# CVMI-Lab/DODA

Measured on AMD Instinct MI355X. Metric: active-voxels/sec fwd+bwd SparseConv U-Net, ScanNet 2cm, higher is better.
Workload: dtype bf16; 1 GPU; cfgs/scannet SparseConv U-Net training step (voxel pooling + fwd + CE + bwd + SGD), 2 cm voxels, 4 scenes/GPU x ~150000 active voxels, random-init weights; global_batch=4, voxels_per_gpu=601279, points_per_gpu=781042, parallelism=dp1, n_classes=20, grad_sync=deferred multi-layer wgrad + bucketed all-reduce, collectives=none (single process), prefetch_gate=off, grad_exchange=no process group

## Files before the change

### doda_amd/csrc/spconv_wwide.hip

```cpp
#include "wgrad_common.hpp"
#include "tilebook.hpp"
#include <string.h>
#include <algorithm>
#include <vector>

namespace {

constexpr int WW_WAVES = 16;
constexpr int WW_MO = (TB_K + WW_WAVES - 1) / WW_WAVES;
constexpr int WW_LIST_BYTES = TB_UMAX * 4;
constexpr int ww_stage_bytes(int ta, int tb) { return TB_T * 32 * tb + (TB_LMAX + 1) * 32 * ta; }
constexpr int WW_STAGE_MAX = ww_stage_bytes(3, 3);
constexpr int WW_SMEM = WW_LIST_BYTES + TB_LIDX_BYTES + WW_STAGE_MAX;
static_assert(WW_SMEM <= 160 * 1024, "one workgroup per CU");
static_assert(TB_T + 1 <= TB_LMAX + 1, "the dense fallback stages 256 rows into the row slots");

struct WwJob {
    const unsigned short *x, *dy;
    const int32_t *tbl;
    const void *tb;
    float *dw, *part;
    int ca, cb, ld, n_rows, nt, ta, tb_, n_sb, P, rpc, accumulate;
    int wg_end, red_end;
    int pad;
};

__device__ __forceinline__ s16x4 ww_tr(unsigned addr) {
    return __builtin_amdgcn_ds_read_tr16_b64_v4i16((__attribute__((address_space(3))) s16x4 *)(uintptr_t)addr);
}
__device__ __forceinline__ bf16x8 ww_frag(unsigned a_lo, unsigned a_hi) {
    const s16x4 lo = ww_tr(a_lo), hi = ww_tr(a_hi);
    return __builtin_bit_cast(bf16x8, __builtin_shufflevector(lo, hi, 0, 1, 2, 3, 4, 5, 6, 7));
}

template <int TA, int TB>
__device__ void ww_body(const WwJob &d, int local, unsigned char *smem) {
    constexpr int RA = 32 * TA, RB = 32 * TB;
    constexpr int CIS = 16 * TA, COS = 16 * TB, SLICE = TB_K * CIS * COS;
    const int tid = threadIdx.x, wid = __builtin_amdgcn_readfirstlane(tid >> 6);
    const int lane = tid & 63, i = lane & 15, g = lane >> 4, q4 = i >> 2, c4 = i & 3;
    const int slice = local / d.P, p = local - slice * d.P;
    const int sa = slice / d.n_sb, sb = slice - sa * d.n_sb;
    const int ca0 = sa * CIS, cb0 = sb * COS;
    const int r_begin = p * d.rpc, r_end = min(d.n_rows, r_begin + d.rpc);
    const int tile_begin = r_begin / TB_T, tile_end = (r_end - 1) / TB_T + 1;
    static_assert(ww_stage_bytes(TA, TB) <= WW_STAGE_MAX, "staging buffers");
    const int32_t *tb_ulist = (const int32_t *)d.tb;
    const uint32_t *tb_lidx = (const uint32_t *)(tb_ulist + (size_t)d.nt * TB_UMAX);
    const int32_t *tb_ucount = (const int32_t *)(tb_lidx + (size_t)d.nt * (TB_LIDX_BYTES / 4));

    int32_t *list_s = reinterpret_cast<int32_t *>(smem);
    const unsigned *lidx_s = reinterpret_cast<const unsigned *>(smem + WW_LIST_BYTES);
    unsigned char *dy_s = smem + WW_LIST_BYTES + TB_LIDX_BYTES;
    unsigned char *rows_s = dy_s + TB_T * RB;
    const unsigned dy_base = (unsigned)(uintptr_t)dy_s, rows_base = (unsigned)(uintptr_t)rows_s;

    f32x4 acc[WW_MO][TA][TB];
#pragma unroll
    for (int m = 0; m < WW_MO; ++m)
#pragma unroll
        for (int a = 0; a < TA; ++a)
#pragma unroll
            for (int b = 0; b < TB; ++b) acc[m][a][b] = (f32x4){0.f, 0.f, 0.f, 0.f};

    auto multiply = [&](bool dense, int only_o, int ks_begin, int ks_end) {
#pragma unroll 1
        for (int ks = ks_begin; ks < ks_end; ++ks) {
            const int r = 32 * ks + 8 * g + q4;
            bf16x8 bf[TB];
#pragma unroll
            for (int b = 0; b < TB; ++b) {
                const unsigned a0 = dy_base + (unsigned)(r * RB + b * 32 + c4 * 8);
                bf[b] = ww_frag(a0, a0 + 4u * RB);
            }
#pragma unroll
            for (int m = 0; m < WW_MO; ++m) {
                const int o = wid + WW_WAVES * m;
                if (o >= TB_K || (dense && o != only_o)) continue;
                unsigned s0, s1;
                if (dense) {
                    s0 = (unsigned)(r + 1);
                    s1 = (unsigned)(r + 5);
                } else {
                    const unsigned *pl = lidx_s + tb_lplane(o) * TB_T;
                    const unsigned sh = tb_lshift(o);
                    s0 = __builtin_amdgcn_ubfe(pl[tb_lpos(r)], sh, 10u);
                    s1 = __builtin_amdgcn_ubfe(pl[tb_lpos(r + 4)], sh, 10u);
                }
                const unsigned x0 = rows_base + s0 * RA + (unsigned)(c4 * 8), x1 = rows_base + s1 * RA + (unsigned)(c4 * 8);
#pragma unroll
                for (int a = 0; a < TA; ++a) {
                    const bf16x8 af = ww_frag(x0 + 32u * a, x1 + 32u * a);
#pragma unroll
                    for (int b = 0; b < TB; ++b)
                        acc[m][a][b] = __builtin_amdgcn_mfma_f32_16x16x32_bf16(af, bf[b], acc[m][a][b], 0, 0, 0);
                }
            }
        }
    };

    for (int e = tid; e < RA / 16; e += 1024) reinterpret_cast<u32x4 *>(rows_s)[e] = (u32x4){0u, 0u, 0u, 0u};
    for (int tile = tile_begin; tile < tile_end; ++tile) {
        const int t0 = tile * TB_T;
        const int ks_begin = max(0, (r_begin - t0) / 32), ks_end = min(TB_T / 32, (r_end - t0 + 31) / 32);
        const int ucount = tb_ucount[tile];
        const bool listed = ucount <= TB_LMAX;
        if (listed) {
            const int e = (tid & 3) * 256 + ((tid >> 7) & 7) * 32 + ((tid >> 2) & 31);
            list_s[e] = tb_ulist[(size_t)tile * TB_UMAX + tid];
            for (int v = tid; v < TB_LIDX_BYTES / 16; v += 1024)
                reinterpret_cast<u32x4 *>(smem + WW_LIST_BYTES)[v] =
                    reinterpret_cast<const u32x4 *>(tb_lidx + (size_t)tile * (TB_LIDX_BYTES / 4))[v];
        }
        for (int v = tid; v < TB_T * (RB / 16); v += 1024) {
            const int t = v / (RB / 16), f = v - t * (RB / 16);
            u32x4 val = (u32x4){0u, 0u, 0u, 0u};
            if (t0 + t < d.n_rows) val = *reinterpret_cast<const u32x4 *>(d.dy + (size_t)(t0 + t) * d.cb + cb0 + f * 8);
            *reinterpret_cast<u32x4 *>(dy_s + t * RB + f * 16) = val;
        }
        doda_sync();
        if (listed) {
            for (int v = tid; v < ucount * (RA / 16); v += 1024) {
                const int e = v / (RA / 16), f = v - e * (RA / 16);
                const int row = list_s[e];
                *reinterpret_cast<u32x4 *>(rows_s + (e + 1) * RA + f * 16) =
                    *reinterpret_cast<const u32x4 *>(d.x + (size_t)row * d.ca + ca0 + f * 8);
            }
            doda_sync();
            multiply(false, 0, ks_begin, ks_end);
            doda_sync();
        } else {
            for (int o = 0; o < TB_K; ++o) {
                for (int v = tid; v < TB_T * (RA / 16); v += 1024) {
                    const int t = v / (RA / 16), f = v - t * (RA / 16);
                    const int row = t0 + t < d.n_rows ? d.tbl[(size_t)o * d.ld + t0 + t] : -1;
                    u32x4 val = (u32x4){0u, 0u, 0u, 0u};
                    if (row >= 0) val = *reinterpret_cast<const u32x4 *>(d.x + (size_t)row * d.ca + ca0 + f * 8);
                    *reinterpret_cast<u32x4 *>(rows_s + (t + 1) * RA + f * 16) = val;
                }
                doda_sync();
                multiply(true, o, ks_begin, ks_end);
                doda_sync();
            }
        }
    }

    float *dst = d.part + (size_t)local * SLICE;
#pragma unroll
    for (int m = 0; m < WW_MO; ++m) {
        const int o = wid + WW_WAVES * m;
        if (o >= TB_K) continue;
#pragma unroll
        for (int a = 0; a < TA; ++a)
#pragma unroll
            for (int b = 0; b < TB; ++b)
#pragma unroll
                for (int r = 0; r < 4; ++r)
                    dst[((size_t)o * CIS + a * 16 + 4 * g + r) * COS + b * 16 + i] = acc[m][a][b][r];
    }
}

__global__ __launch_bounds__(1024) void wgrad_wide(const WwJob *__restrict__ jobs, int n_jobs) {
    __shared__ __attribute__((aligned(16))) unsigned char smem[WW_SMEM];
    const int j = find_job<WwJob, &WwJob::wg_end>(jobs, n_jobs, (int)blockIdx.x);
    const WwJob d = jobs[j];
    const int local = (int)blockIdx.x - (j == 0 ? 0 : jobs[j - 1].wg_end);
#define WW_CASE(A, B) if (d.ta == A && d.tb_ == B) { ww_body<A, B>(d, local, smem); return; }
    WW_SHAPES(WW_CASE)
#undef WW_CASE
}

__global__ __launch_bounds__(256) void wgrad_wide_reduce(const WwJob *__restrict__ jobs, int n_jobs) {
    const int j = find_job<WwJob, &WwJob::red_end>(jobs, n_jobs, (int)blockIdx.x);
    const WwJob d = jobs[j];
    const int CIS = 16 * d.ta, COS = 16 * d.tb_, SLICE = TB_K * CIS * COS;
    wgrad_fold((int)blockIdx.x - (j == 0 ? 0 : jobs[j - 1].red_end), d.P, (long long)TB_K * d.ca * d.cb / 4, SLICE / 4,
               reinterpret_cast<float4 *>(d.dw), d.accumulate, [&](long long q) {
        const long long e = 4 * q;
        const int co = (int)(e % d.cb), ci = (int)((e / d.cb) % d.ca), o = (int)(e / ((long long)d.ca * d.cb));
        const int slice = (ci / CIS) * d.n_sb + co / COS;
        return reinterpret_cast<const float4 *>(d.part + ((size_t)slice * d.P) * SLICE + ((size_t)o * CIS + ci % CIS) * COS + co % COS);
    });
}

}

namespace doda_wwide {

Plan plan(const doda_wgrad_job *jobs, const std::vector<int> &idx) {
    Plan pl;
    pl.n = (int)idx.size();
    std::vector<int> order;
    for (int k = 0; k < pl.n; ++k) order.push_back(k);
    std::stable_sort(order.begin(), order.end(), [&](int a, int b) { return jobs[idx[a]].n_rows > jobs[idx[b]].n_rows; });
    std::vector<WwJob> desc;
    for (int kk : order) {
        const doda_wgrad_job &j = jobs[idx[kk]];
        WwJob d;
        d.x = (const unsigned short *)j.a; d.dy = (const unsigned short *)j.b; d.tbl = j.tbl; d.tb = j.tilebook;
        d.dw = j.dw;
        d.ca = j.ca; d.cb = j.cb; d.ld = j.ld; d.n_rows = j.n_rows; d.nt = (j.n_rows + TB_T - 1) / TB_T;
        const WideGeo g = wwide_geo(j, doda_wgrad::switches());
        d.ta = g.ta; d.tb_ = g.tb; d.rpc = g.rpc; d.P = g.P;
        d.n_sb = j.cb / (16 * d.tb_);
        d.accumulate = (j.flags & DODA_WGRAD_ACCUMULATE) ? 1 : 0;
        d.part = (float *)(uintptr_t)pl.partial_bytes;
        pl.partial_bytes += g.partial_bytes;
        pl.wgs += g.blocks;
        d.wg_end = pl.wgs;
        pl.red_blocks += doda_wgrad::reduce_blocks((long long)TB_K * j.ca * j.cb / 4, d.P);
        d.red_end = pl.red_blocks;
        d.pad = 0;
        desc.push_back(d);
    }
    pl.desc_bytes = desc.size() * sizeof(WwJob);
    pl.desc.resize(pl.desc_bytes);
    if (pl.desc_bytes) memcpy(pl.desc.data(), desc.data(), pl.desc_bytes);
    return pl;
}

size_t desc_bytes_per_job() { return sizeof(WwJob); }

void write_desc(const Plan &p, char *part, void *desc) {
    if (p.desc_bytes) memcpy(desc, p.desc.data(), p.desc_bytes);
    WwJob *d = (WwJob *)desc;
    for (int k = 0; k < p.n; ++k) d[k].part = (float *)(part + (uintptr_t)d[k].part);
}

int launch(const Plan &p, const void *desc_dev, hipStream_t s) {
    doda_wgrad::trace("wgrad_wide", p.wgs, 1024, p.n);
    hipLaunchKernelGGL(wgrad_wide, dim3(p.wgs), dim3(1024), 0, s, (const WwJob *)desc_dev, p.n);
    doda_wgrad::trace("wgrad_wide_reduce", p.red_blocks, 256, p.n);
    hipLaunchKernelGGL(wgrad_wide_reduce, dim3(p.red_blocks), dim3(256), 0, s, (const WwJob *)desc_dev, p.n);
    return doda_check_launch();
}

}
```

### doda_amd/csrc/wgrad_common.hpp

```cpp
#pragma once
#include "wgrad_backends.hpp"

typedef float f32x4 __attribute__((ext_vector_type(4)));
typedef short s16x4 __attribute__((ext_vector_type(4)));
typedef __bf16 bf16x8 __attribute__((ext_vector_type(8)));
typedef unsigned int u32x4 __attribute__((ext_vector_type(4)));

namespace {

template <class J, int J::*END>
__device__ __forceinline__ int find_job(const J *jobs, int n_jobs, int blk) {
    int lo = 0, hi = n_jobs - 1;
    while (lo < hi) {
        const int mid = (lo + hi) >> 1;
        if (blk < jobs[mid].*END) hi = mid; else lo = mid + 1;
    }
    return lo;
}

__device__ __forceinline__ bf16x8 pack_hi16(const f32x4 &d0, const f32x4 &d1) {
    u32x4 r;
    r[0] = __builtin_amdgcn_perm(__float_as_uint(d0[1]), __float_as_uint(d0[0]), 0x07060302u);
    r[1] = __builtin_amdgcn_perm(__float_as_uint(d0[3]), __float_as_uint(d0[2]), 0x07060302u);
    r[2] = __builtin_amdgcn_perm(__float_as_uint(d1[1]), __float_as_uint(d1[0]), 0x07060302u);
    r[3] = __builtin_amdgcn_perm(__float_as_uint(d1[3]), __float_as_uint(d1[2]), 0x07060302u);
    return __builtin_bit_cast(bf16x8, r);
}

template <class Src>
__device__ __forceinline__ void wgrad_fold(int blk, int R, long long n_quad, long long stride, float4 *dw, int accumulate,
                                           Src src) {
    __shared__ float4 part[256];
    const int RL = doda_wgrad::reduce_lanes(R), EL = 256 / RL;
    const int el = (int)threadIdx.x % EL, rl = (int)threadIdx.x / EL;
    const long long q = (long long)blk * EL + el;
    float4 s = make_float4(0.f, 0.f, 0.f, 0.f);
    if (q < n_quad) {
        const float4 *p = src(q);
        for (int r = rl; r < R; r += RL) {
            const float4 v = p[(long long)r * stride];
            s.x += v.x; s.y += v.y; s.z += v.z; s.w += v.w;
        }
    }
    part[rl * EL + el] = s;
    doda_sync();
    if (rl == 0 && q < n_quad) {
        float4 t = part[el];
        for (int r = 1; r < RL; ++r) {
            const float4 v = part[r * EL + el];
            t.x += v.x; t.y += v.y; t.z += v.z; t.w += v.w;
        }
        if (accumulate) {
            const float4 old = dw[q];
            t.x += old.x; t.y += old.y; t.z += old.z; t.w += old.w;
        }
        dw[q] = t;
    }
}

}
```

Measured before the change: 138.3 million voxels/s.

## Pipeline wide wgrad tiles with async LDS DMA, double-buffered lists and faster job lookup

Gathered input rows for the next tile are now fetched into LDS with global_load_lds DMA requests interleaved with the current tile's MFMA loop. The tile lists are double-buffered, and the row area is split from both ends so two tiles' rows can coexist. The next tile's dy and lidx are prefetched into registers. It also adds a TA==1 loop order that reuses A fragments, a ballot-based job lookup, cheaper unsigned index math in the reduce, and a 4-way unrolled fold loop. The goal is to hide gather latency and cut barriers, at the cost of more registers, inline asm that manipulates m0, and a more intricate synchronization scheme.

```diff
diff --git a/doda_amd/csrc/spconv_wwide.hip b/doda_amd/csrc/spconv_wwide.hip
--- a/doda_amd/csrc/spconv_wwide.hip
+++ b/doda_amd/csrc/spconv_wwide.hip
@@ -9,11 +9,16 @@
 constexpr int WW_WAVES = 16;
 constexpr int WW_MO = (TB_K + WW_WAVES - 1) / WW_WAVES;
 constexpr int WW_LIST_BYTES = TB_UMAX * 4;
-constexpr int ww_stage_bytes(int ta, int tb) { return TB_T * 32 * tb + (TB_LMAX + 1) * 32 * ta; }
-constexpr int WW_STAGE_MAX = ww_stage_bytes(3, 3);
-constexpr int WW_SMEM = WW_LIST_BYTES + TB_LIDX_BYTES + WW_STAGE_MAX;
-static_assert(WW_SMEM <= 160 * 1024, "one workgroup per CU");
-static_assert(TB_T + 1 <= TB_LMAX + 1, "the dense fallback stages 256 rows into the row slots");
+constexpr int WW_SMEM = 160 * 1024;
+template <int TA, int TB>
+struct WwLds {
+    static constexpr int RA = 32 * TA, RB = 32 * TB;
+    static constexpr int LIST = 0, LIDX = 2 * WW_LIST_BYTES, DY = LIDX + TB_LIDX_BYTES, ROWS = DY + TB_T * RB;
+    static constexpr int SLOTS = (WW_SMEM - ROWS) / RA;
+    static constexpr int NDY = (TB_T * (RB / 16) + 1023) / 1024;
+    static_assert(SLOTS >= TB_LMAX + 1, "a full list fits the row area");
+    static_assert(TB_T + 1 <= SLOTS, "the dense fallback stages 256 rows into the row slots");
+};
 
 struct WwJob {
     const unsigned short *x, *dy;
@@ -33,9 +38,32 @@
     return __builtin_bit_cast(bf16x8, __builtin_shufflevector(lo, hi, 0, 1, 2, 3, 4, 5, 6, 7));
 }
 
+#define WW_GLOBAL __attribute__((address_space(1)))
+template <class T>
+__device__ __forceinline__ WW_GLOBAL T *ww_global(T *p) { return (WW_GLOBAL T *)p; }
+typedef const WW_GLOBAL u32x4 *ww_g128;
+
+__device__ __forceinline__ void ww_dma16(unsigned lds_base, const WW_GLOBAL void *src) {
+    unsigned keep;
+    asm volatile("s_mov_b32 %0, m0\n\t"
+                 "s_mov_b32 m0, %1\n\t"
+                 "s_nop 0\n\t"
+                 "global_load_lds_dwordx4 %2, off\n\t"
+                 "s_mov_b32 m0, %0"
+                 : "=&s"(keep) : "s"(lds_base), "v"(src) : "memory");
+}
+__device__ __forceinline__ void ww_dma_drain() { asm volatile("s_waitcnt vmcnt(0)" ::: "memory"); }
+
+__device__ __forceinline__ int ww_tid() {
+    int t = (int)threadIdx.x;
+    asm volatile("" : "+v"(t));
+    return t;
+}
+
 template <int TA, int TB>
 __device__ void ww_body(const WwJob &d, int local, unsigned char *smem) {
-    constexpr int RA = 32 * TA, RB = 32 * TB;
+    typedef WwLds<TA, TB> L;
+    constexpr int RA = L::RA, RB = L::RB, NDY = L::NDY;
     constexpr int CIS = 16 * TA, COS = 16 * TB, SLICE = TB_K * CIS * COS;
     const int tid = threadIdx.x, wid = __builtin_amdgcn_readfirstlane(tid >> 6);
     const int lane = tid & 63, i = lane & 15, g = lane >> 4, q4 = i >> 2, c4 = i & 3;
@@ -44,16 +72,19 @@
     const int ca0 = sa * CIS, cb0 = sb * COS;
     const int r_begin = p * d.rpc, r_end = min(d.n_rows, r_begin + d.rpc);
     const int tile_begin = r_begin / TB_T, tile_end = (r_end - 1) / TB_T + 1;
-    static_assert(ww_stage_bytes(TA, TB) <= WW_STAGE_MAX, "staging buffers");
     const int32_t *tb_ulist = (const int32_t *)d.tb;
     const uint32_t *tb_lidx = (const uint32_t *)(tb_ulist + (size_t)d.nt * TB_UMAX);
     const int32_t *tb_ucount = (const int32_t *)(tb_lidx + (size_t)d.nt * (TB_LIDX_BYTES / 4));
-
-    int32_t *list_s = reinterpret_cast<int32_t *>(smem);
-    const unsigned *lidx_s = reinterpret_cast<const unsigned *>(smem + WW_LIST_BYTES);
-    unsigned char *dy_s = smem + WW_LIST_BYTES + TB_LIDX_BYTES;
-    unsigned char *rows_s = dy_s + TB_T * RB;
-    const unsigned dy_base = (unsigned)(uintptr_t)dy_s, rows_base = (unsigned)(uintptr_t)rows_s;
+    const WW_GLOBAL unsigned short *gx = ww_global(d.x), *gdy = ww_global(d.dy);
+    const WW_GLOBAL int32_t *gtbl = ww_global(d.tbl);
+
+    const unsigned *lidx_s = reinterpret_cast<const unsigned *>(smem + L::LIDX);
+    unsigned char *dy_s = smem + L::DY;
+    unsigned char *rows_s = smem + L::ROWS;
+    const unsigned dy_base = (unsigned)(uintptr_t)dy_s;
+    const auto list_of = [&](int tile) { return reinterpret_cast<int32_t *>(smem + L::LIST + (tile & 1) * WW_LIST_BYTES); };
+    const auto rows_of = [&](int tile, int ucount) { return rows_s + ((tile & 1) ? (L::SLOTS - (ucount + 1)) * RA : 0); };
+    const auto list_e = [](int t) { return (t & 3) * 256 + ((t >> 7) & 7) * 32 + ((t >> 2) & 31); };
 
     f32x4 acc[WW_MO][TA][TB];
 #pragma unroll
@@ -63,20 +94,49 @@
 #pragma unroll
             for (int b = 0; b < TB; ++b) acc[m][a][b] = (f32x4){0.f, 0.f, 0.f, 0.f};
 
-    auto multiply = [&](bool dense, int only_o, int ks_begin, int ks_end) {
+    u32x4 p_lidx = (u32x4){0u, 0u, 0u, 0u}, p_dy[NDY];
+    const auto load_p1 = [&](int tile) {
+        const int tl = ww_tid();
+        if (tl < TB_LIDX_BYTES / 16) p_lidx = reinterpret_cast<ww_g128>(ww_global(tb_lidx) + (size_t)tile * (TB_LIDX_BYTES / 4))[tl];
+#pragma unroll
+        for (int k = 0; k < NDY; ++k) {
+            const int v = tl + 1024 * k, t = v / (RB / 16), f = v - t * (RB / 16);
+            p_dy[k] = (u32x4){0u, 0u, 0u, 0u};
+            if (v < TB_T * (RB / 16) && tile * TB_T + t < d.n_rows)
+                p_dy[k] = *reinterpret_cast<ww_g128>(gdy + (size_t)(tile * TB_T + t) * d.cb + cb0 + f * 8);
+        }
+    };
+    const auto store_p1 = [&]() {
+        const int tl = ww_tid();
+        if (tl < TB_LIDX_BYTES / 16) reinterpret_cast<u32x4 *>(smem + L::LIDX)[tl] = p_lidx;
+#pragma unroll
+        for (int k = 0; k < NDY; ++k) {
+            const int v = tl + 1024 * k;
+            if (v < TB_T * (RB / 16)) reinterpret_cast<u32x4 *>(dy_s)[v] = p_dy[k];
+        }
+    };
+    const auto request_rows = [&](const int32_t *list, unsigned char *rows, int n, int &vb) {
+        const int v = vb + (ww_tid() & 63);
+        if (v < n) {
+            const int e = v / (RA / 16), f = v - e * (RA / 16);
+            ww_dma16(__builtin_amdgcn_readfirstlane((unsigned)(uintptr_t)rows + (unsigned)(RA + 16 * vb)),
+                     gx + (size_t)list[e] * d.ca + ca0 + f * 8);
+        }
+        vb += 1024;
+    };
+
+    auto multiply = [&](bool dense, int only_o, int ks_begin, int ks_end, unsigned rows_base, const int32_t *next_list,
+                        unsigned char *next_rows, int n_next) {
+        int vb = 64 * wid;
 #pragma unroll 1
         for (int ks = ks_begin; ks < ks_end; ++ks) {
+            if (vb < n_next) request_rows(next_list, next_rows, n_next, vb);
             const int r = 32 * ks + 8 * g + q4;
-            bf16x8 bf[TB];
-#pragma unroll
-            for (int b = 0; b < TB; ++b) {
+            const auto b_frag = [&](int b) {
                 const unsigned a0 = dy_base + (unsigned)(r * RB + b * 32 + c4 * 8);
-                bf[b] = ww_frag(a0, a0 + 4u * RB);
-            }
-#pragma unroll
-            for (int m = 0; m < WW_MO; ++m) {
-                const int o = wid + WW_WAVES * m;
-                if (o >= TB_K || (dense && o != only_o)) continue;
+                return ww_frag(a0, a0 + 4u * RB);
+            };
+            const auto a_rows = [&](int o, unsigned *x0, unsigned *x1) {
                 unsigned s0, s1;
                 if (dense) {
                     s0 = (unsigned)(r + 1);
@@ -87,65 +147,116 @@
                     s0 = __builtin_amdgcn_ubfe(pl[tb_lpos(r)], sh, 10u);
                     s1 = __builtin_amdgcn_ubfe(pl[tb_lpos(r + 4)], sh, 10u);
                 }
-                const unsigned x0 = rows_base + s0 * RA + (unsigned)(c4 * 8), x1 = rows_base + s1 * RA + (unsigned)(c4 * 8);
-#pragma unroll
-                for (int a = 0; a < TA; ++a) {
-                    const bf16x8 af = ww_frag(x0 + 32u * a, x1 + 32u * a);
-#pragma unroll
-                    for (int b = 0; b < TB; ++b)
-                        acc[m][a][b] = __builtin_amdgcn_mfma_f32_16x16x32_bf16(af, bf[b], acc[m][a][b], 0, 0, 0);
+                *x0 = rows_base + s0 * RA + (unsigned)(c4 * 8);
+                *x1 = rows_base + s1 * RA + (unsigned)(c4 * 8);
+            };
+            if constexpr (TA == 1) {
+                bf16x8 af[WW_MO];
+                bool own[WW_MO];
+#pragma unroll
+                for (int m = 0; m < WW_MO; ++m) {
+                    const int o = wid + WW_WAVES * m;
+                    own[m] = o < TB_K && !(dense && o != only_o);
+                    if (!own[m]) continue;
+                    unsigned x0, x1;
+                    a_rows(o, &x0, &x1);
+                    af[m] = ww_frag(x0, x1);
+                }
+#pragma unroll
+                for (int b = 0; b < TB; ++b) {
+                    const bf16x8 bf = b_frag(b);
+#pragma unroll
+                    for (int m = 0; m < WW_MO; ++m)
+                        if (own[m]) acc[m][0][b] = __builtin_amdgcn_mfma_f32_16x16x32_bf16(af[m], bf, acc[m][0][b], 0, 0, 0);
+                }
+            } else {
+                bf16x8 bf[TB];
+#pragma unroll
+                for (int b = 0; b < TB; ++b) bf[b] = b_frag(b);
+#pragma unroll
+                for (int m = 0; m < WW_MO; ++m) {
+                    const int o = wid + WW_WAVES * m;
+                    if (o >= TB_K || (dense && o != only_o)) continue;
+                    unsigned x0, x1;
+                    a_rows(o, &x0, &x1);
+#pragma unroll
+                    for (int a = 0; a < TA; ++a) {
+                        const bf16x8 af = ww_frag(x0 + 32u * a, x1 + 32u * a);
+#pragma unroll
+                        for (int b = 0; b < TB; ++b)
+                            acc[m][a][b] = __builtin_amdgcn_mfma_f32_16x16x32_bf16(af, bf[b], acc[m][a][b], 0, 0, 0);
+                    }
                 }
             }
         }
+        while (vb < n_next) request_rows(next_list, next_rows, n_next, vb);
     };
 
-    for (int e = tid; e < RA / 16; e += 1024) reinterpret_cast<u32x4 *>(rows_s)[e] = (u32x4){0u, 0u, 0u, 0u};
+    bool have_p1 = false;
+    bool have_rows = false;
+    const auto count_of = [&](int tile) { return tile < tile_end ? ww_global(tb_ucount)[tile + (ww_tid() >> 31)] : TB_LMAX + 1; };
+    int ucount = count_of(tile_begin), ucount1 = count_of(tile_begin + 1);
     for (int tile = tile_begin; tile < tile_end; ++tile) {
         const int t0 = tile * TB_T;
         const int ks_begin = max(0, (r_begin - t0) / 32), ks_end = min(TB_T / 32, (r_end - t0 + 31) / 32);
-        const int ucount = tb_ucount[tile];
+        const bool next = tile + 1 < tile_end;
         const bool listed = ucount <= TB_LMAX;
-        if (listed) {
-            const int e = (tid & 3) * 256 + ((tid >> 7) & 7) * 32 + ((tid >> 2) & 31);
-            list_s[e] = tb_ulist[(size_t)tile * TB_UMAX + tid];
-            for (int v = tid; v < TB_LIDX_BYTES / 16; v += 1024)
-                reinterpret_cast<u32x4 *>(smem + WW_LIST_BYTES)[v] =
-                    reinterpret_cast<const u32x4 *>(tb_lidx + (size_t)tile * (TB_LIDX_BYTES / 4))[v];
-        }
-        for (int v = tid; v < TB_T * (RB / 16); v += 1024) {
-            const int t = v / (RB / 16), f = v - t * (RB / 16);
-            u32x4 val = (u32x4){0u, 0u, 0u, 0u};
-            if (t0 + t < d.n_rows) val = *reinterpret_cast<const u32x4 *>(d.dy + (size_t)(t0 + t) * d.cb + cb0 + f * 8);
-            *reinterpret_cast<u32x4 *>(dy_s + t * RB + f * 16) = val;
-        }
+        if (!have_p1) {
+            load_p1(tile);
+            const int tl = ww_tid();
+            list_of(tile)[list_e(tl)] = tb_ulist[(size_t)tile * TB_UMAX + tl];
+            if (next) list_of(tile + 1)[list_e(tl)] = tb_ulist[(size_t)(tile + 1) * TB_UMAX + tl];
+        }
+        store_p1();
         doda_sync();
         if (listed) {
-            for (int v = tid; v < ucount * (RA / 16); v += 1024) {
-                const int e = v / (RA / 16), f = v - e * (RA / 16);
-                const int row = list_s[e];
-                *reinterpret_cast<u32x4 *>(rows_s + (e + 1) * RA + f * 16) =
-                    *reinterpret_cast<const u32x4 *>(d.x + (size_t)row * d.ca + ca0 + f * 8);
+            unsigned char *rows = rows_of(tile, ucount);
+            if (!have_rows) {
+                const int tl = ww_tid();
+                if (tl < RA / 16) reinterpret_cast<u32x4 *>(rows)[tl] = (u32x4){0u, 0u, 0u, 0u};
+                const int32_t *list = list_of(tile);
+                for (int vb = 64 * wid; vb < ucount * (RA / 16);) request_rows(list, rows, ucount * (RA / 16), vb);
+                ww_dma_drain();
+                doda_sync();
             }
+            int next_list = -1;
+            if (next) load_p1(tile + 1);
+            const int count2 = count_of(tile + 2);
+            if (tile + 2 < tile_end) next_list = ww_global(tb_ulist)[(size_t)(tile + 2) * TB_UMAX + ww_tid()];
+            const bool stage = next && ucount1 <= TB_LMAX && ucount + ucount1 + 2 <= L::SLOTS;
+            unsigned char *rows1 = rows_of(tile + 1, ucount1);
+            if (stage && ww_tid() < RA / 16) reinterpret_cast<u32x4 *>(rows1)[ww_tid()] = (u32x4){0u, 0u, 0u, 0u};
+            multiply(false, 0, ks_begin, ks_end, (unsigned)(uintptr_t)rows, list_of(tile + 1), rows1,
+                     stage ? ucount1 * (RA / 16) : 0);
+            ww_dma_drain();
             doda_sync();
-            multiply(false, 0, ks_begin, ks_end);
-            doda_sync();
+            if (tile + 2 < tile_end) list_of(tile)[list_e(ww_tid())] = next_list;
+            have_p1 = next;
+            have_rows = stage;
+            ucount = ucount1;
+            ucount1 = count2;
         } else {
             for (int o = 0; o < TB_K; ++o) {
-                for (int v = tid; v < TB_T * (RA / 16); v += 1024) {
+                for (int v = ww_tid(); v < TB_T * (RA / 16); v += 1024) {
                     const int t = v / (RA / 16), f = v - t * (RA / 16);
-                    const int row = t0 + t < d.n_rows ? d.tbl[(size_t)o * d.ld + t0 + t] : -1;
+                    const int row = t0 + t < d.n_rows ? gtbl[(size_t)o * d.ld + t0 + t] : -1;
                     u32x4 val = (u32x4){0u, 0u, 0u, 0u};
-                    if (row >= 0) val = *reinterpret_cast<const u32x4 *>(d.x + (size_t)row * d.ca + ca0 + f * 8);
+                    if (row >= 0) val = *reinterpret_cast<ww_g128>(gx + (size_t)row * d.ca + ca0 + f * 8);
                     *reinterpret_cast<u32x4 *>(rows_s + (t + 1) * RA + f * 16) = val;
                 }
                 doda_sync();
-                multiply(true, o, ks_begin, ks_end);
+                multiply(true, o, ks_begin, ks_end, (unsigned)(uintptr_t)rows_s, nullptr, nullptr, 0);
                 doda_sync();
             }
+            have_p1 = false;
+            have_rows = false;
+            ucount = ucount1;
+            ucount1 = count_of(tile + 2);
         }
     }
 
-    float *dst = d.part + (size_t)local * SLICE;
+    WW_GLOBAL float *dst = ww_global(d.part) + (size_t)local * SLICE;
+    const int ti = ww_tid() & 15, tg = (ww_tid() & 63) >> 4;
 #pragma unroll
     for (int m = 0; m < WW_MO; ++m) {
         const int o = wid + WW_WAVES * m;
@@ -156,30 +267,48 @@
             for (int b = 0; b < TB; ++b)
 #pragma unroll
                 for (int r = 0; r < 4; ++r)
-                    dst[((size_t)o * CIS + a * 16 + 4 * g + r) * COS + b * 16 + i] = acc[m][a][b][r];
+                    dst[((size_t)o * CIS + a * 16 + 4 * tg + r) * COS + b * 16 + ti] = acc[m][a][b][r];
     }
+}
+
+template <int WwJob::*END>
+__device__ __forceinline__ int ww_find(const WwJob *jobs, int n_jobs, int blk, int *first) {
+    if (n_jobs > 64) {
+        const int j = find_job<WwJob, END>(jobs, n_jobs, blk);
+        *first = j == 0 ? 0 : jobs[j - 1].*END;
+        return j;
+    }
+    const int lane = (int)threadIdx.x & 63;
+    const int end = lane < n_jobs ? jobs[lane].*END : 0x7fffffff;
+    const int j = __builtin_amdgcn_readfirstlane(__popcll(__ballot(end <= blk)));
+    *first = __builtin_amdgcn_readfirstlane(__shfl(end, j > 0 ? j - 1 : 0, 64));
+    if (j == 0) *first = 0;
+    return j;
 }
 
 __global__ __launch_bounds__(1024) void wgrad_wide(const WwJob *__restrict__ jobs, int n_jobs) {
     __shared__ __attribute__((aligned(16))) unsigned char smem[WW_SMEM];
-    const int j = find_job<WwJob, &WwJob::wg_end>(jobs, n_jobs, (int)blockIdx.x);
+    int first;
+    const int j = ww_find<&WwJob::wg_end>(jobs, n_jobs, (int)blockIdx.x, &first);
     const WwJob d = jobs[j];
-    const int local = (int)blockIdx.x - (j == 0 ? 0 : jobs[j - 1].wg_end);
+    const int local = (int)blockIdx.x - first;
 #define WW_CASE(A, B) if (d.ta == A && d.tb_ == B) { ww_body<A, B>(d, local, smem); return; }
     WW_SHAPES(WW_CASE)
 #undef WW_CASE
 }
 
 __global__ __launch_bounds__(256) void wgrad_wide_reduce(const WwJob *__restrict__ jobs, int n_jobs) {
-    const int j = find_job<WwJob, &WwJob::red_end>(jobs, n_jobs, (int)blockIdx.x);
+    int first;
+    const int j = ww_find<&WwJob::red_end>(jobs, n_jobs, (int)blockIdx.x, &first);
     const WwJob d = jobs[j];
     const int CIS = 16 * d.ta, COS = 16 * d.tb_, SLICE = TB_K * CIS * COS;
-    wgrad_fold((int)blockIdx.x - (j == 0 ? 0 : jobs[j - 1].red_end), d.P, (long long)TB_K * d.ca * d.cb / 4, SLICE / 4,
+    wgrad_fold((int)blockIdx.x - first, d.P, (long long)TB_K * d.ca * d.cb / 4, SLICE / 4,
                reinterpret_cast<float4 *>(d.dw), d.accumulate, [&](long long q) {
-        const long long e = 4 * q;
-        const int co = (int)(e % d.cb), ci = (int)((e / d.cb) % d.ca), o = (int)(e / ((long long)d.ca * d.cb));
-        const int slice = (ci / CIS) * d.n_sb + co / COS;
-        return reinterpret_cast<const float4 *>(d.part + ((size_t)slice * d.P) * SLICE + ((size_t)o * CIS + ci % CIS) * COS + co % COS);
+        const unsigned e = 4u * (unsigned)q, row = e / (unsigned)d.cb;
+        const int co = (int)(e - row * (unsigned)d.cb), o = (int)(row / (unsigned)d.ca), ci = (int)(row - (unsigned)o * (unsigned)d.ca);
+        const int sa = ci / CIS, sb = co / COS;
+        const int slice = sa * d.n_sb + sb;
+        return reinterpret_cast<const float4 *>(d.part + ((size_t)slice * d.P) * SLICE + ((size_t)o * CIS + (ci - sa * CIS)) * COS + (co - sb * COS));
     });
 }
 
diff --git a/doda_amd/csrc/wgrad_common.hpp b/doda_amd/csrc/wgrad_common.hpp
--- a/doda_amd/csrc/wgrad_common.hpp
+++ b/doda_amd/csrc/wgrad_common.hpp
@@ -37,9 +37,14 @@
     float4 s = make_float4(0.f, 0.f, 0.f, 0.f);
     if (q < n_quad) {
         const float4 *p = src(q);
-        for (int r = rl; r < R; r += RL) {
-            const float4 v = p[(long long)r * stride];
-            s.x += v.x; s.y += v.y; s.z += v.z; s.w += v.w;
+        for (int r = rl; r < R; r += 4 * RL) {
+            float4 v[4];
+#pragma unroll
+            for (int k = 0; k < 4; ++k)
+                if (r + k * RL < R) v[k] = p[(long long)(r + k * RL) * stride];
+#pragma unroll
+            for (int k = 0; k < 4; ++k)
+                if (r + k * RL < R) { s.x += v[k].x; s.y += v[k].y; s.z += v[k].z; s.w += v[k].w; }
         }
     }
     part[rl * EL + el] = s;
```

Result: no change. 139.4 million voxels/s, median of 6 (+0.8%).
